# rlawhdrhs/Vision-Transformer-OpenCL

Hardware: AMD Instinct MI355X
Metric: images/sec ViT-B/16 224² fp32 @batch256; % MFMA roofline; top-1 match (higher is better)
Workload: dtype f32; 1 GPU; ViT-B/16 224x224 fp32 forward, batch 256 per GPU, synthetic weights and images (BASELINE.json configs[1]); batch_per_gpu=256, global_batch=256, parallelism=dp1, lanes_per_gpu=1, prune_last_layer=False, ln_fold=True, device=AMD Radeon Graphics, arch=gfx950:sramecc+:xnack-, compute_units=256, clock_mhz=2400

## Files before the change

### vision-transformer-opencl_amd/csrc/vit_gemm_common.hpp

```cpp
#pragma once
#include <hip/hip_runtime.h>

#include <type_traits>

#include "vit_hip_kernels.h"
#include "vit_split3.hpp"

namespace vitgemm {


typedef float f32x16 __attribute__((ext_vector_type(16)));
typedef float f32x4 __attribute__((ext_vector_type(4)));
typedef float f32x2 __attribute__((ext_vector_type(2)));
typedef unsigned u32x4 __attribute__((ext_vector_type(4)));

constexpr int KALIGN = 32;

enum { A_DENSE = 0, A_PATCHES = 1 };
enum { EPI_BIAS_LN = 3, EPI_BIAS_GELU_LN = 4, EPI_RESIDUAL_STATS = 5, EPI_BIAS_QGELU_LN = 7  };
constexpr bool epi_is_fold(int epi) { return epi == EPI_BIAS_LN || epi == EPI_BIAS_GELU_LN || epi == EPI_BIAS_QGELU_LN; }
constexpr bool epi_is_gelu(int epi) { return epi == VITHIP_EPI_BIAS_GELU || epi == EPI_BIAS_GELU_LN; }
constexpr bool epi_is_qgelu(int epi) { return epi == VITHIP_EPI_BIAS_QGELU || epi == EPI_BIAS_QGELU_LN; }

template <int... EPIS, typename F>
// ... 159 lines not shown
#pragma unroll
    for (int v = 0; v < NP; ++v) t[v] = f32x2{__builtin_amdgcn_rcpf(t[v].x), __builtin_amdgcn_rcpf(t[v].y)};
    __builtin_amdgcn_sched_barrier(0);
#pragma unroll
    for (int v = 0; v < NP; ++v) y[v] = y[v] * t[v];
}
__device__ __forceinline__ void quick_gelu_x8(float (&y)[8]) {
    f32x2 yy[4];
#pragma unroll
    for (int v = 0; v < 4; ++v) yy[v] = f32x2{y[2 * v], y[2 * v + 1]};
    quick_gelu_lockstep<4>(yy);
#pragma unroll
    for (int v = 0; v < 4; ++v) y[2 * v] = yy[v].x, y[2 * v + 1] = yy[v].y;
}

__device__ __forceinline__ int xcd_remap(int bid, int nwg) {
    const int q = nwg >> 3, rem = nwg & 7;
    const int xcd = bid & 7, idx = bid >> 3;
    const int base = xcd < rem ? xcd * (q + 1) : rem * (q + 1) + (xcd - rem) * q;
    return base + idx;
}

__device__ __forceinline__ void tile_coords(int tile, int tiles_m, int tiles_n, int group_m, int &tm, int &tn) {
    const int per_group = group_m * tiles_n;
    const int g = tile / per_group, in_g = tile - g * per_group;
    const int first = g * group_m;
    const int rows = tiles_m - first < group_m ? tiles_m - first : group_m;
    tn = in_g / rows;
    tm = first + (in_g - tn * rows);
}


enum { ARITH_F32 = 0, ARITH_SPLIT3 = 1 };
typedef __bf16 bf16x8 __attribute__((ext_vector_type(8)));
typedef __bf16 bf16x4 __attribute__((ext_vector_type(4)));
typedef unsigned u32x2 __attribute__((ext_vector_type(2)));
constexpr int SPLIT_BK = 16;
constexpr int SPLIT_LD = 28;
using vitsplit::SPLIT_TERM_A;
using vitsplit::SPLIT_TERM_W;
using vitsplit::bf16_to_f32;
using vitsplit::split3_piece;
using vitsplit::split3_piece2;
using vitsplit::split3_piece8;
__device__ __forceinline__ void split3_store(float *row, int kc, f32x4 x) {
#pragma unroll
    for (int piece = 0; piece < 3; ++piece) *reinterpret_cast<u32x2 *>(row + piece * 8 + kc / 2) = split3_piece(x, piece);
}

constexpr int WIMG_ROWS = 128;
constexpr int WIMG_BLOCK_BYTES = 3 * WIMG_ROWS * SPLIT_BK * 2;
constexpr int SPLIT_LD_SW = 32;
__device__ __forceinline__ int split_swizzle(int row) { return 2 * ((row & 3) ^ ((row >> 2) & 3)) + ((row >> 3) & 1); }
__device__ __forceinline__ int split_sw_offset(int row, int s) { return row * SPLIT_LD_SW + 4 * (s ^ split_swizzle(row)); }
template <int TM, int TN, int NS, typename Restage>
__device__ __forceinline__ void split3_step(f32x16 (&acc)[TM][TN], const float *As, const float *Bs, Restage &&restage) {
    bf16x8 a[TM][3], b[TN][3];
#pragma unroll
    for (int o = 0; o < 3; ++o) {
        const int pa = SPLIT_TERM_A[o], pb = SPLIT_TERM_W[o];
#pragma unroll
        for (int i = 0; i < TM; ++i) a[i][pa] = *reinterpret_cast<const bf16x8 *>(As + i * 32 * SPLIT_LD + pa * 8);
#pragma unroll
        for (int j = 0; j < TN; ++j) b[j][pb] = *reinterpret_cast<const bf16x8 *>(Bs + j * 32 * SPLIT_LD + pb * 8);
    }
    __builtin_amdgcn_sched_barrier(0);
    constexpr int NM = 6 * TM * TN, NR = NM / 2 > 0 ? NM / 2 : 1;
#pragma unroll
    for (int idx = 0; idx < NM; ++idx) {
        const int t = idx / (TM * TN), i = (idx / TN) % TM, j = idx % TN;
        acc[i][j] = __builtin_amdgcn_mfma_f32_32x32x16_bf16(a[i][SPLIT_TERM_A[t]], b[j][SPLIT_TERM_W[t]], acc[i][j], 0, 0, 0);
        if (idx < NR) {
            const int slot_before = (idx * NS) / NR, slot_after = ((idx + 1) * NS) / NR;
            if (slot_after > slot_before) {
                __builtin_amdgcn_sched_barrier(0);
#pragma unroll
                for (int q = slot_before; q < slot_after; ++q) restage(q);
                __builtin_amdgcn_sched_barrier(0);
            }
        }
    }
}

struct Split3PfRead { int w, piece, behind; };
constexpr int SPLIT_PF_BARRIER = 15;
constexpr Split3PfRead SPLIT_PF_READS[6] = {{0, 0, 15}, {1, 0, 16}, {1, 2, 17}, {0, 2, 18}, {0, 1, 19}, {1, 1, 20}};
struct Split3SlotsFine {
    static constexpr int N = 21;
    static constexpr int at(int q) {
        constexpr int gap[N] = {0, 1, 2, 3, 4, 4, 5, 6, 7, 8, 8, 9, 10, 12, 13, 1, 5, 9, 2, 6, 11};
        return gap[q];
    }
};
constexpr int split3_last_use(int w, int piece, int per_term) {
    int last = -1;
    for (int t = 0; t < 6; ++t)
        if ((w ? SPLIT_TERM_W[t] : SPLIT_TERM_A[t]) == piece) last = (t + 1) * per_term - 1;
    return last;
}
constexpr bool split3_pf_schedule_ok(int per_term) {
    for (int q = 0; q < Split3SlotsFine::N; ++q)
        if (Split3SlotsFine::at(q) < 0 || Split3SlotsFine::at(q) > SPLIT_PF_BARRIER) return false;
    bool seen[2][3] = {};
    for (int e = 0; e < 6; ++e) {
        const Split3PfRead rd = SPLIT_PF_READS[e];
        if (rd.behind < SPLIT_PF_BARRIER || rd.behind >= 6 * per_term) return false;
        if (rd.piece != 0 && rd.behind < split3_last_use(rd.w, rd.piece, per_term)) return false;
        if (e > 0 && rd.behind < SPLIT_PF_READS[e - 1].behind) return false;
        seen[rd.w][rd.piece] = true;
    }
    for (int w = 0; w < 2; ++w)
        for (int pc = 0; pc < 3; ++pc)
            if (!seen[w][pc]) return false;
    return true;
}
template <int TM, int TN>
struct Split3Frags {
    bf16x8 a[TM][3], b[TN][3];
    bf16x8 a_hn[TM], b_hn[TN];
};
template <int TM, int TN, bool NEXT>
__device__ __forceinline__ void split3_read_piece(Split3Frags<TM, TN> &f, const float *As, const float *Bs, const int (&poff)[3], int e) {
    const Split3PfRead rd = SPLIT_PF_READS[e];
    if (rd.w == 0) {
#pragma unroll
        for (int i = 0; i < TM; ++i) {
            const bf16x8 v = *reinterpret_cast<const bf16x8 *>(As + i * 32 * SPLIT_LD_SW + poff[rd.piece]);
            if (NEXT && rd.piece == 0) f.a_hn[i] = v;
            else f.a[i][rd.piece] = v;
        }
    } else {
#pragma unroll
        for (int j = 0; j < TN; ++j) {
            const bf16x8 v = *reinterpret_cast<const bf16x8 *>(Bs + j * 32 * SPLIT_LD_SW + poff[rd.piece]);
            if (NEXT && rd.piece == 0) f.b_hn[j] = v;
            else f.b[j][rd.piece] = v;
        }
    }
}
template <int TM, int TN>
__device__ __forceinline__ void split3_read_cold(Split3Frags<TM, TN> &f, const float *As, const float *Bs, const int (&poff)[3]) {
#pragma unroll
    for (int e = 0; e < 6; ++e) split3_read_piece<TM, TN, false>(f, As, Bs, poff, e);
}
struct Split3NoHook {
    __device__ __forceinline__ void operator()() const {}
};
template <int TM, int TN, bool PF, typename Restage, typename Sync, typename Landed = Split3NoHook>
__device__ __forceinline__ void split3_step_pf(f32x16 (&acc)[TM][TN], Split3Frags<TM, TN> &f, const float *An, const float *Bn,
                                               const int (&poff)[3], Restage &&restage, Sync &&sync, Landed &&landed = Landed{}) {
    constexpr int NM = 6 * TM * TN;
    static_assert(NM == 24, "the schedule table is laid out for 2 x 2 accumulators");
    static_assert(split3_pf_schedule_ok(TM * TN),
                  "restage writes in front of the barrier, reads of the other buffer behind it and behind the last use of what they overwrite");
    landed();
    __builtin_amdgcn_sched_barrier(0);
#pragma unroll
    for (int idx = 0; idx < NM; ++idx) {
        const int t = idx / (TM * TN), i = (idx / TN) % TM, j = idx % TN;
        acc[i][j] = __builtin_amdgcn_mfma_f32_32x32x16_bf16(f.a[i][SPLIT_TERM_A[t]], f.b[j][SPLIT_TERM_W[t]], acc[i][j], 0, 0, 0);
        __builtin_amdgcn_sched_barrier(0);
#pragma unroll
        for (int q = 0; q < Split3SlotsFine::N; ++q)
            if (Split3SlotsFine::at(q) == idx) restage(q);
        if (idx == SPLIT_PF_BARRIER) sync();
        if constexpr (PF) {
#pragma unroll
            for (int e = 0; e < 6; ++e)
                if (SPLIT_PF_READS[e].behind == idx) split3_read_piece<TM, TN, true>(f, An, Bn, poff, e);
        }
        __builtin_amdgcn_sched_barrier(0);
    }
    if constexpr (PF) {
#pragma unroll
        for (int i = 0; i < TM; ++i) f.a[i][0] = f.a_hn[i];
#pragma unroll
        for (int j = 0; j < TN; ++j) f.b[j][0] = f.b_hn[j];
    }
}

template <int TN, int TM = 1>
struct FoldOperands {
    float colsum[TN];
    const f32x2 *rows;
    float rstd[TM][16], mean[TM];
    bool preloaded;
};
template <int TN, int TM>
__device__ __forceinline__ void fold_preload(FoldOperands<TN, TM> &fold, const float *ln_rows, int M, int m_tile, int r, int h) {
#pragma unroll
    for (int i = 0; i < TM; ++i) {
        const int mr = m_tile + i * 32 + r;
        fold.mean[i] = ln_rows[2 * (size_t)(mr < M ? mr : M - 1) + 1];
#pragma unroll
        for (int v = 0; v < 16; ++v) {
            const int m = m_tile + i * 32 + 4 * h + (v & 3) + 8 * (v >> 2);
            fold.rstd[i][v] = ln_rows[2 * (size_t)(m < M ? m : M - 1)];
        }
    }
    fold.preloaded = true;
}
__device__ __forceinline__ float fold_center(float acc, float mean, float colsum) { return __builtin_fmaf(-mean, colsum, acc); }
__device__ __forceinline__ float fold_scale(float centered, float rstd, float bias) { return __builtin_fmaf(rstd, centered, bias); }

template <int BM, int BN, int WM, int WN, int EPI, int AMODE>
__device__ __forceinline__ void epilogue_store(const GemmParams &p, const f32x16 (&acc)[WM / 32][WN / 32],
                                               const float (&bias_r)[WN / 32], int m0, int n0, int wm, int wn,
                                               int r, int h, const FoldOperands<WN / 32, WM / 32> &fold = FoldOperands<WN / 32, WM / 32>{}) {
    constexpr int TM = WM / 32, TN = WN / 32;
    constexpr bool FOLD = epi_is_fold(EPI);
    constexpr bool GELU = epi_is_gelu(EPI), QGELU = epi_is_qgelu(EPI);
    constexpr int ST_NT = 2;
    const bool interior = (m0 + BM <= p.M) && (n0 + BN <= p.N);
    if (interior) {
        if constexpr (FOLD) {
            const __amdgpu_buffer_rsrc_t c_rsrc = __builtin_amdgcn_make_buffer_rsrc(p.C, 0, 0x7fffffff, 0x00020000);
            const bool center = p.ln_colsum != nullptr;
            auto rstd_of_block = [&](int i, float (&dst)[16]) __attribute__((always_inline)) {
#pragma unroll
                for (int g = 0; g < 4; ++g) {
                    const int lr = wm * WM + i * 32 + 4 * h + 8 * g;
#pragma unroll
                    for (int e = 0; e < 4; ++e) dst[4 * g + e] = fold.preloaded ? fold.rstd[i][4 * g + e] : fold.rows[lr + e].x;
                }
            };
            auto scale_and_store = [&](int i, const f32x16 (&src)[TN], const float (&row_rstd)[16]) __attribute__((always_inline)) {
                const int mb = m0 + wm * WM + i * 32 + 4 * h;
#pragma unroll
                for (int j = 0; j < TN; ++j) {
                    const int n = n0 + wn * WN + j * 32 + r;
                    const int c_off = (mb * p.ldc + n) * 4, c_row = p.ldc * 4;
#pragma unroll
                    for (int half = 0; half < 2; ++half) {
                        float y[8];
#pragma unroll
                        for (int q = 0; q < 8; ++q) y[q] = fold_scale(src[j][half * 8 + q], row_rstd[half * 8 + q], bias_r[j]);
                        if constexpr (GELU) gelu_erf_x8(y);
                        if constexpr (QGELU) quick_gelu_x8(y);
#pragma unroll
                        for (int q = 0; q < 8; ++q) {
                            const int v = half * 8 + q;
                            __builtin_amdgcn_raw_buffer_store_b32(__builtin_bit_cast(unsigned, y[q]), c_rsrc, c_off, ((v & 3) + 8 * (v >> 2)) * c_row, ST_NT);
                        }
                    }
                }
            };
            if (center) {
                float b_op[TN];
#pragma unroll
                for (int j = 0; j < TN; ++j) b_op[j] = h == 0 ? fold.colsum[j] : 0.0f;
#pragma unroll
                for (int i = 0; i < TM; ++i) {
                    const float mean = fold.preloaded ? fold.mean[i] : fold.rows[wm * WM + i * 32 + r].y;
                    const float a_op = h == 0 ? -mean : 0.0f;
                    f32x16 centered[TN];
#pragma unroll
                    for (int j = 0; j < TN; ++j) centered[j] = __builtin_amdgcn_mfma_f32_32x32x2f32(a_op, b_op[j], acc[i][j], 0, 0, 0);
                    float row_rstd[16];
                    rstd_of_block(i, row_rstd);
                    scale_and_store(i, centered, row_rstd);
// ... 215 lines not shown
```

### vision-transformer-opencl_amd/csrc/vit_gemm_persistent.hip

```cpp
#include "vit_device.hpp"
#include "vit_gemm_common.hpp"

namespace vitgemm {

constexpr int PBK = 32;
constexpr int PLD = PBK + 4;
constexpr int SK_HEADER_BYTES = 4096, SK_MAX_OWNERS = 1000, SK_STAT_TAKEN = 1016, SK_STAT_RECOMPUTED = 1017;

template <int BM, int BN, int WM, int WN, int EPI, bool STAMP = false, bool SK = false, int DBG = 0, int ARITH = ARITH_F32,
          bool WIMG = false>
__global__ __launch_bounds__(256, 2) void gemm_f32_nt_persistent_kernel(const GemmParams p) {
    constexpr bool SPLIT = ARITH == ARITH_SPLIT3;
    static_assert(!SPLIT || DBG == 0, "switch-off builds are fp32 only");
    static_assert(!WIMG || (SPLIT && BM == WIMG_ROWS && BN == WIMG_ROWS), "the weight image feeds the 128x128 split walk");
    constexpr bool PIPE = WIMG && EPI != VITHIP_EPI_BIAS_RESIDUAL && EPI != EPI_RESIDUAL_STATS;
    constexpr int PBK = SPLIT ? SPLIT_BK : vitgemm::PBK;
    constexpr int PLD = WIMG ? SPLIT_LD_SW : SPLIT ? SPLIT_LD : vitgemm::PLD;
    constexpr int ROWS_PER_PASS = 256 / (PBK / 4);
    constexpr int WGN = BN / WN;
    constexpr int TM = WM / 32, TN = WN / 32;
    constexpr int A_CHUNKS = BM * (PBK / 4) / 256;
    constexpr int B_CHUNKS = BN * (PBK / 4) / 256;
    constexpr int NC = PBK / 8;
    constexpr int NS = A_CHUNKS + B_CHUNKS;
    constexpr int W_CHUNKS = 3;
    constexpr int NL = WIMG ? A_CHUNKS + W_CHUNKS : NS;
    static_assert(!WIMG || (A_CHUNKS == 2 && BM * 2 == 256 && BN * 2 == 256), "WIMG: one 8-deep half row of A and of W per thread");
    constexpr int NM = 4 * TM * TN;
    static_assert((BM / WM) * WGN == 4, "4 waves per workgroup");

    __shared__ __attribute__((aligned(16))) float lds[2 * (BM + BN) * PLD];
    __shared__ int sk_decision;
    constexpr bool FOLD = epi_is_fold(EPI);
    __shared__ __attribute__((aligned(16))) f32x2 fold_rows_lds[FOLD ? 2 * BM : 2];
    static_assert(!FOLD || BM == 128, "one 16-byte lane copy of 64 lanes = 128 rows");
    float *const As0 = lds;
    float *const Bs0 = lds + 2 * BM * PLD;

    const int tid = threadIdx.x;
    const int lane = tid & 63, wave = tid >> 6;
    const int r = lane & 31, h = lane >> 5;
    const int wm = wave / WGN, wn = wave % WGN;

    unsigned long long st0 = 0, st_rt0 = 0, st_loop0 = 0, st_epi = 0;
    [[maybe_unused]] unsigned long long st_frag = 0, st_top = 0, st_landed = 0;
    auto stamp_top = [&]() __attribute__((always_inline)) {
        if constexpr (STAMP && WIMG) st_top = __builtin_amdgcn_s_memtime();
    };
    auto stamp_landed = [&]() __attribute__((always_inline)) {
        if constexpr (STAMP && WIMG) {
            __builtin_amdgcn_s_waitcnt(0xC07F);
            st_landed = __builtin_amdgcn_s_memtime();
        }
    };
    auto stamp_step = [&]() __attribute__((always_inline)) {
        if constexpr (STAMP && WIMG) st_frag += st_landed - st_top;
    };
    if constexpr (STAMP) {
        st0 = __builtin_amdgcn_s_memtime();
        st_rt0 = __builtin_amdgcn_s_memrealtime();
    }

    const int total = p.tiles_m * p.tiles_n;
    const int nwg = gridDim.x;
    const int first = xcd_remap(blockIdx.x, nwg);
    if (first >= total) return;
    const int nk = p.K / PBK;

    const int full = total / nwg, R = total - full * nwg;
    const int x = SK ? p.sk_x : 0;
    const int H = nwg - R;
    const bool owner = first < R;
    const int npre = (x > 0 && !owner && R > 0) ? (R - (first - R) + H - 1) / H : 0;
    const int pstart = (SK && p.sk_late) ? full : 0, fstart = (SK && p.sk_late) ? 0 : npre;
    const int nseg = npre + full + (owner ? 1 : 0);
    bool took = false;
    struct Seg { int tile, k0, k1, in, out; };
    auto get_seg = [&](int i) -> Seg {
        Seg g;
        if (i >= pstart && i < pstart + npre) {
            const int o = (first - R) + (i - pstart) * H;
            g.tile = full * nwg + o; g.k0 = 0; g.k1 = x; g.in = -1; g.out = o;
        } else if (i < npre + full) {
            g.tile = first + (i - fstart) * nwg; g.k0 = 0; g.k1 = nk; g.in = -1; g.out = -1;
        } else {
            g.tile = first + full * nwg; g.k0 = took ? x : 0; g.k1 = nk; g.in = took ? first : -1; g.out = -1;
        }
        return g;
    };

    const int ld_row = tid / (PBK / 4);
    const int ld_kc = (tid % (PBK / 4)) * 4;
    const int sw_row = tid >> 1, sw_half = tid & 1;
    int wr_off[3];
#pragma unroll
    for (int pl = 0; pl < 3; ++pl) wr_off[pl] = WIMG ? split_sw_offset(sw_row, 2 * pl + sw_half) : 0;
    const __amdgpu_buffer_rsrc_t a_rsrc = __builtin_amdgcn_make_buffer_rsrc(const_cast<float *>(p.A), 0, 0x7fffffff, 0x00020000);
    const __amdgpu_buffer_rsrc_t w_rsrc =
        __builtin_amdgcn_make_buffer_rsrc(const_cast<void *>(WIMG ? p.w_split : static_cast<const void *>(p.W)), 0, 0x7fffffff, 0x00020000);
    int a_src[A_CHUNKS];
    int b_src[WIMG ? W_CHUNKS : B_CHUNKS];
    f32x4 a_stage[A_CHUNKS], b_stage[B_CHUNKS];
    u32x4 w_stage[WIMG ? W_CHUNKS : 1];

    auto set_sources = [&](int tile) {
        int tm, tn;
        tile_coords(tile, p.tiles_m, p.tiles_n, p.group_m, tm, tn);
        if constexpr (WIMG) {
            int m = tm * BM + sw_row;
            m = m < p.M ? m : p.M - 1;
#pragma unroll
            for (int i = 0; i < A_CHUNKS; ++i) a_src[i] = (m * p.lda + 8 * sw_half + 4 * i) * 4;
#pragma unroll
            for (int q = 0; q < W_CHUNKS; ++q) b_src[q] = tn * nk * WIMG_BLOCK_BYTES + (q * 256 + tid) * 16;
            return;
        }
#pragma unroll
        for (int i = 0; i < A_CHUNKS; ++i) {
            int m = tm * BM + ld_row + i * ROWS_PER_PASS;
            m = m < p.M ? m : p.M - 1;
            a_src[i] = (m * p.lda + ld_kc) * 4;
        }
#pragma unroll
        for (int i = 0; i < B_CHUNKS; ++i) {
            int n = tn * BN + ld_row + i * ROWS_PER_PASS;
            n = n < p.N ? n : p.N - 1;
            b_src[i] = (n * p.ldw + ld_kc) * 4;
        }
    };
    auto load_bias = [&](int n0, float (&dst)[TN]) {
#pragma unroll
        for (int j = 0; j < TN; ++j) {
            const int n = n0 + wn * WN + j * 32 + r;
            dst[j] = n < p.N ? p.bias[n] : 0.0f;
        }
    };

    int *const sk_flags = reinterpret_cast<int *>(p.sk_ws);
    const int SK_PARKED = (p.sk_gen << 2) | 1, SK_WITHDRAWN = (p.sk_gen << 2) | 2;
    int steps = 0;
    auto decide = [&]() {
        if (tid == 0) {
            int *const f = sk_flags + first;
            int v = __hip_atomic_load(f, __ATOMIC_RELAXED, __HIP_MEMORY_SCOPE_AGENT);
            while (v != SK_PARKED) {
                int expected = v;
                if (__hip_atomic_compare_exchange_strong(f, &expected, SK_WITHDRAWN, __ATOMIC_RELAXED, __ATOMIC_RELAXED, __HIP_MEMORY_SCOPE_AGENT)) {
                    v = SK_WITHDRAWN;
                    break;
                }
                v = expected;
            }
            if (v == SK_PARKED) __hip_atomic_store(f, 0, __ATOMIC_RELAXED, __HIP_MEMORY_SCOPE_AGENT);
            __hip_atomic_fetch_add(sk_flags + (v == SK_PARKED ? SK_STAT_TAKEN : SK_STAT_RECOMPUTED), 1, __ATOMIC_RELAXED, __HIP_MEMORY_SCOPE_AGENT);
            sk_decision = v == SK_PARKED;
        }
        __syncthreads();
        took = __builtin_amdgcn_readfirstlane(sk_decision) != 0;
        if (took) steps -= x;
    };

    int seg_l = 0, k_l, kend_l;
    {
        const Seg g = get_seg(0);
        set_sources(g.tile);
        k_l = g.k0;
        kend_l = g.k1;
    }
    auto advance_load_cursor = [&]() {
        if (++k_l == kend_l) {
            if (++seg_l < nseg) {
                if (SK && owner && x > 0 && seg_l == nseg - 1) decide();
                const Seg g = get_seg(seg_l);
                set_sources(g.tile);
                k_l = g.k0;
                kend_l = g.k1;
            } else {
                k_l = kend_l - 1;
            }
        }
    };
    auto load_step = [&]() {
        const int k0 = k_l * PBK;
#pragma unroll
        for (int i = 0; i < A_CHUNKS; ++i) a_stage[i] = __builtin_bit_cast(f32x4, __builtin_amdgcn_raw_buffer_load_b128(a_rsrc, a_src[i], k0 * 4, 0));
        if constexpr (WIMG) {
#pragma unroll
            for (int q = 0; q < W_CHUNKS; ++q) w_stage[q] = __builtin_amdgcn_raw_buffer_load_b128(w_rsrc, b_src[q], k_l * WIMG_BLOCK_BYTES, 0);
            return;
        }
#pragma unroll
        for (int i = 0; i < B_CHUNKS; ++i) b_stage[i] = __builtin_bit_cast(f32x4, __builtin_amdgcn_raw_buffer_load_b128(w_rsrc, b_src[i], k0 * 4, 0));
    };
    auto stage_write = [&](float *row, f32x4 v) __attribute__((always_inline)) {
        if constexpr (SPLIT) split3_store(row, ld_kc, v);
        else *reinterpret_cast<f32x4 *>(row + ld_kc) = v;
    };
    auto write_a_plane = [&](float *As, int pl) __attribute__((always_inline)) {
        *reinterpret_cast<u32x4 *>(As + wr_off[pl]) = split3_piece8(a_stage[0], a_stage[1], pl);
    };
    auto write_w_plane = [&](float *Bs, int pl) __attribute__((always_inline)) { *reinterpret_cast<u32x4 *>(Bs + wr_off[pl]) = w_stage[pl]; };
    auto store_step = [&](int buf) {
        float *As = As0 + buf * BM * PLD, *Bs = Bs0 + buf * BN * PLD;
        if constexpr (WIMG) {
#pragma unroll
            for (int pl = 0; pl < 3; ++pl) {
                write_a_plane(As, pl);
                write_w_plane(Bs, pl);
            }
            return;
        }
#pragma unroll
        for (int i = 0; i < A_CHUNKS; ++i) stage_write(As + (ld_row + i * ROWS_PER_PASS) * PLD, a_stage[i]);
#pragma unroll
        for (int i = 0; i < B_CHUNKS; ++i) stage_write(Bs + (ld_row + i * ROWS_PER_PASS) * PLD, b_stage[i]);
    };
    auto restage_slot = [&](int q, int buf, int k0) {
        if (q < A_CHUNKS) {
            float *As = As0 + buf * BM * PLD;
            if (DBG != 5 && DBG != 6) stage_write(As + (ld_row + q * ROWS_PER_PASS) * PLD, a_stage[q]);
            if (DBG != 2 && DBG != 6) a_stage[q] = __builtin_bit_cast(f32x4, __builtin_amdgcn_raw_buffer_load_b128(a_rsrc, a_src[q], k0 * 4, 0));
        } else {
            const int qb = q - A_CHUNKS;
            float *Bs = Bs0 + buf * BN * PLD;
            if (DBG != 5 && DBG != 6) stage_write(Bs + (ld_row + qb * ROWS_PER_PASS) * PLD, b_stage[qb]);
            if (DBG != 2 && DBG != 6) b_stage[qb] = __builtin_bit_cast(f32x4, __builtin_amdgcn_raw_buffer_load_b128(w_rsrc, b_src[qb], k0 * 4, 0));
        }
    };

    u32x4 a_plane;
    auto restage_fine = [&](int q, int buf, int k0) {
        if (q <= 12) {
            const int pl = q / 5, sub = q % 5;
            auto quarter = [&](int s4) __attribute__((always_inline)) {
                f32x4 &x = a_stage[s4 >> 1];
                const int o = 2 * (s4 & 1);
                f32x2 xx = {x[o], x[o + 1]};
                unsigned pc = split3_piece2(xx, pl);
                asm volatile("" : "+v"(pc), "+v"(xx));
                x[o] = xx[0];
                x[o + 1] = xx[1];
                a_plane[s4] = pc;
            };
            if (pl < 2 && sub < 4) quarter(sub);
            else if (pl == 2 && sub < 2) {
                quarter(2 * sub);
                quarter(2 * sub + 1);
            } else *reinterpret_cast<u32x4 *>(As0 + buf * BM * PLD + wr_off[pl]) = a_plane;
        } else if (q <= 14) {
            a_stage[q - 13] = __builtin_bit_cast(f32x4, __builtin_amdgcn_raw_buffer_load_b128(a_rsrc, a_src[q - 13], k0 * 4, 0));
        } else if (q <= 17) {
            write_w_plane(Bs0 + buf * BN * PLD, q - 15);
        } else {
            w_stage[q - 18] = __builtin_amdgcn_raw_buffer_load_b128(w_rsrc, b_src[q - 18], (k0 / PBK) * WIMG_BLOCK_BYTES, 0);
        }
    };
    auto restage_any = [&](int q, int buf, int k0) __attribute__((always_inline)) {
        restage_fine(q, buf, k0);
    };

    const int a_frag_off = WIMG ? (wm * WM + r) * PLD : (wm * WM + r) * PLD + h * 4;
    const int b_frag_off = WIMG ? (wn * WN + r) * PLD : (wn * WN + r) * PLD + h * 4;
    int frag_poff[3];
#pragma unroll
    for (int pc = 0; pc < 3; ++pc) frag_poff[pc] = WIMG ? split_sw_offset(r, 2 * pc + h) - r * PLD : 0;
    f32x4 af[2][TM], bf[2][TN];
    auto read_frags = [&](int buf, int c, int set) {
        if constexpr (SPLIT) return;
        const float *As = As0 + buf * BM * PLD + a_frag_off + c * 8;
        const float *Bs = Bs0 + buf * BN * PLD + b_frag_off + c * 8;
#pragma unroll
        for (int i = 0; i < TM; ++i) af[set][i] = *reinterpret_cast<const f32x4 *>(As + i * 32 * PLD);
#pragma unroll
        for (int j = 0; j < TN; ++j) bf[set][j] = *reinterpret_cast<const f32x4 *>(Bs + j * 32 * PLD);
    };

    f32x16 acc[TM][TN];
    constexpr int SC_SYS = 0x11;
    auto slot_rsrc = [&](int o) {
        return __builtin_amdgcn_make_buffer_rsrc(reinterpret_cast<char *>(p.sk_ws) + SK_HEADER_BYTES + (size_t)o * (BM * BN * 4), 0, BM * BN * 4, 0x00020000);
    };
    auto park = [&](int o) {
        const __amdgpu_buffer_rsrc_t rs = slot_rsrc(o);
#pragma unroll
        for (int i = 0; i < TM; ++i)
#pragma unroll
            for (int j = 0; j < TN; ++j)
#pragma unroll
                for (int q4 = 0; q4 < 4; ++q4) {
                    f32x4 v;
#pragma unroll
                    for (int e = 0; e < 4; ++e) v[e] = acc[i][j][4 * q4 + e];
                    __builtin_amdgcn_raw_buffer_store_b128(__builtin_bit_cast(u32x4, v), rs, tid * 16,
                                                           ((i * TN + j) * 4 + q4) * 4096, SC_SYS);
                }
        asm volatile("s_waitcnt vmcnt(0)" ::: "memory");
        __syncthreads();
        if (tid == 0) {
            int cur = __hip_atomic_load(sk_flags + o, __ATOMIC_RELAXED, __HIP_MEMORY_SCOPE_AGENT);
            for (;;) {
                if (cur == SK_WITHDRAWN) {
                    __hip_atomic_store(sk_flags + o, 0, __ATOMIC_RELAXED, __HIP_MEMORY_SCOPE_AGENT);
                    break;
                }
                int expected = cur;
                if (__hip_atomic_compare_exchange_strong(sk_flags + o, &expected, SK_PARKED, __ATOMIC_RELAXED, __ATOMIC_RELAXED, __HIP_MEMORY_SCOPE_AGENT)) break;
                cur = expected;
            }
        }
    };
    auto unpark = [&](int o) {
        const __amdgpu_buffer_rsrc_t rs = slot_rsrc(o);
#pragma unroll
        for (int i = 0; i < TM; ++i)
#pragma unroll
            for (int j = 0; j < TN; ++j)
#pragma unroll
                for (int q4 = 0; q4 < 4; ++q4) {
                    const f32x4 v = __builtin_bit_cast(f32x4, __builtin_amdgcn_raw_buffer_load_b128(rs, tid * 16, ((i * TN + j) * 4 + q4) * 4096, SC_SYS));
#pragma unroll
                    for (int e = 0; e < 4; ++e) acc[i][j][4 * q4 + e] = v[e];
                }
        __builtin_amdgcn_s_waitcnt(0x0F70);
    };

    int seg_c = 0, k_c, kend_c, m0, n0, out_c;
    [[maybe_unused]] int seg_k0 = 0;
    float bias_r[TN];
    FoldOperands<TN, TM> fold{};
    [[maybe_unused]] int fold_buf = 0;
    auto begin_segment = [&](int i) {
        const Seg g = get_seg(i);
        int tm, tn;
        tile_coords(g.tile, p.tiles_m, p.tiles_n, p.group_m, tm, tn);
        m0 = tm * BM;
        n0 = tn * BN;
        k_c = g.k0;
        seg_k0 = g.k0;
        kend_c = g.k1;
        out_c = g.out;
        if (g.out < 0) load_bias(n0, bias_r);
        if constexpr (FOLD) {
            if (g.out < 0) {
#pragma unroll
                for (int j = 0; j < TN; ++j) {
                    const int n = n0 + wn * WN + j * 32 + r;
                    fold.colsum[j] = (p.ln_colsum && n < p.N) ? p.ln_colsum[n] : 0.0f;
                }
                if (wave == 0) {
                    const int left = p.M - m0 < BM ? p.M - m0 : BM;
                    const __amdgpu_buffer_rsrc_t rr = __builtin_amdgcn_make_buffer_rsrc(const_cast<float *>(p.ln_rows) + (size_t)m0 * 2, 0, left * 8, 0x00020000);
                    const unsigned dst = (unsigned)(size_t)(fold_rows_lds + fold_buf * BM);
                    asm volatile("s_mov_b32 m0, %0\n\ts_nop 0\n\tbuffer_load_dwordx4 %1, %2, 0 offen lds" ::"s"(dst), "v"(lane * 16), "s"(rr) : "memory", "m0");
                }
                fold.rows = fold_rows_lds + fold_buf * BM;
                fold_buf ^= 1;
            }
        }
        if (SK && g.in >= 0) {
            unpark(g.in);
        } else {
#pragma unroll
            for (int ii = 0; ii < TM; ++ii)
#pragma unroll
                for (int jj = 0; jj < TN; ++jj)
#pragma unroll
                    for (int v = 0; v < 16; ++v) acc[ii][jj][v] = 0.0f;
        }
    };
    begin_segment(0);

    for (int i = 0; i < nseg; ++i) {
        const Seg g = get_seg(i);
        steps += g.k1 - g.k0;
    }
    load_step();
    advance_load_cursor();
    store_step(0);
    load_step();
    advance_load_cursor();
    __syncthreads();
    read_frags(0, 0, 0);
    if (DBG == 4) read_frags(0, 1, 1);
    (void)af; (void)bf;

    auto end_segment = [&]() {
        unsigned long long e0 = 0;
        if constexpr (STAMP) e0 = __builtin_amdgcn_s_memtime();
        if (SK && out_c >= 0) park(out_c);
        else if (DBG != 1 || p.M < 0) {
            if constexpr (EPI == EPI_RESIDUAL_STATS) epilogue_store_residual_stats<BM, BN, WM, WN>(p, acc, bias_r, m0, n0, wm, wn, r, h);
            else epilogue_store<BM, BN, WM, WN, EPI, A_DENSE>(p, acc, bias_r, m0, n0, wm, wn, r, h, fold);
        }
        if constexpr (STAMP) st_epi += __builtin_amdgcn_s_memtime() - e0;
        if (++seg_c < nseg) begin_segment(seg_c);
    };
    auto fold_rows_landed = [&]() {
        if constexpr (FOLD) {
            if (out_c < 0) {
                constexpr int FOLD_WAIT = 2 * NL, FOLD_MIN_STEPS = 4;
                static_assert(FOLD_WAIT <= 63, "vmcnt is a 6-bit count on gfx950");
                static_assert((FOLD_MIN_STEPS - 1) * NL >= FOLD_WAIT + NL, "the copy must be older than the loads the wait leaves in flight");
                if (kend_c - seg_k0 >= FOLD_MIN_STEPS) asm volatile("s_waitcnt vmcnt(%0)" ::"n"(FOLD_WAIT) : "memory");
                else asm volatile("s_waitcnt vmcnt(0)" ::: "memory");
            }
        }
    };

    if constexpr (STAMP) st_loop0 = __builtin_amdgcn_s_memtime();
    int cur = 0;
    if constexpr (PIPE) {
        Split3Frags<TM, TN> frags;
        auto tile_a = [&](int buf) { return As0 + buf * BM * PLD + a_frag_off; };
        auto tile_b = [&](int buf) { return Bs0 + buf * BN * PLD + b_frag_off; };
        auto step = [&](auto prefetch) __attribute__((always_inline)) {
            constexpr bool PF = decltype(prefetch)::value;
            const int k_ahead = k_l * PBK;
            split3_step_pf<TM, TN, PF>(acc, frags, tile_a(cur ^ 1), tile_b(cur ^ 1), frag_poff,
                [&](int q) __attribute__((always_inline)) { restage_any(q, cur ^ 1, k_ahead); }, [] { __syncthreads(); }, stamp_landed);
            stamp_step();
            stamp_top();
            advance_load_cursor();
            cur ^= 1;
            ++k_c;
        };
        for (;;) {
            stamp_top();
            split3_read_cold<TM, TN>(frags, tile_a(cur), tile_b(cur), frag_poff);
            while (k_c + 1 < kend_c) step(std::true_type{});
            fold_rows_landed();
            step(std::false_type{});
            end_segment();
            if (seg_c >= nseg) break;
        }
    } else
    for (int g = 0; g < steps; ++g) {
        const int k_ahead = k_l * PBK;
        if (k_c + 1 == kend_c) fold_rows_landed();
        if constexpr (WIMG) {
            Split3Frags<TM, TN> frags;
            stamp_top();
            split3_read_cold<TM, TN>(frags, As0 + cur * BM * PLD + a_frag_off, Bs0 + cur * BN * PLD + b_frag_off, frag_poff);
            split3_step_pf<TM, TN, false>(acc, frags, nullptr, nullptr, frag_poff,
                [&](int q) __attribute__((always_inline)) { restage_fine(q, cur ^ 1, k_ahead); }, [] {}, stamp_landed);
            stamp_step();
            advance_load_cursor();
            __syncthreads();
        } else if constexpr (SPLIT) {
            split3_step<TM, TN, NS>(acc, As0 + cur * BM * PLD + a_frag_off, Bs0 + cur * BN * PLD + b_frag_off,
                                    [&](int q) __attribute__((always_inline)) { restage_slot(q, cur ^ 1, k_ahead); });
            advance_load_cursor();
            __syncthreads();
        } else
#pragma unroll
        for (int c = 0; c < NC; ++c) {
            if (c + 1 < NC && DBG != 4) read_frags(cur, c + 1, (c + 1) & 1);
            if (c == NC - 1) {
                if (DBG != 3) __syncthreads();
                if (DBG != 4) read_frags(cur ^ 1, 0, NC & 1);
            }
            __builtin_amdgcn_sched_barrier(0);
#pragma unroll
            for (int idx = 0; idx < NM; ++idx) {
                const int s2 = idx / (TM * TN), i = (idx / TN) % TM, j = idx % TN;
                acc[i][j] = __builtin_amdgcn_mfma_f32_32x32x2f32(af[c & 1][i][s2], bf[c & 1][j][s2], acc[i][j], 0, 0, 0);
                if (c == 0) {
                    const int slot_before = (idx * NS) / NM, slot_after = ((idx + 1) * NS) / NM;
                    if (slot_after > slot_before) {
                        __builtin_amdgcn_sched_barrier(0);
#pragma unroll
                        for (int q = slot_before; q < slot_after; ++q) restage_slot(q, cur ^ 1, k_ahead);
                        __builtin_amdgcn_sched_barrier(0);
                    }
                }
            }
            if (c == 0) advance_load_cursor();
        }
        cur ^= 1;

        if (++k_c == kend_c) end_segment();
    }
    if constexpr (STAMP) {
        const unsigned long long c3 = __builtin_amdgcn_s_memtime(), r3 = __builtin_amdgcn_s_memrealtime();
        if (tid == 0) {
            unsigned long long *d = p.dbg + (size_t)blockIdx.x * 8;
            d[0] = st0; d[1] = st_loop0; d[2] = st_epi; d[3] = c3; d[4] = WIMG ? st_frag : st_rt0; d[5] = r3;
            d[6] = (unsigned long long)nseg; d[7] = (unsigned long long)steps;
        }
    }
}

static int persistent_wgs() { return 2 * vitdev::current_cus(); }

int persistent_piece_steps(int M, int N, int K, int slots, int wgs, int kstep) {
    if (wgs <= 0) wgs = persistent_wgs();
    if (wgs <= 0) return 0;
    const int total = ((M + 127) / 128) * ((N + 127) / 128);
    const int nwg = total < wgs ? total : wgs;
    const int full = total / nwg, R = total - full * nwg, nk = K / PBK;
    if (full < 1 || R <= 0 || R >= nwg || R > slots || R > SK_MAX_OWNERS) return 0;
    const int c = (R + (nwg - R) - 1) / (nwg - R);
    const int x = nk / (c + 1);
    return (x >= 4 && nk - c * x >= 8) ? x * (PBK / kstep) : 0;
}

template <int BM, int BN, int WM, int WN, int ARITH = ARITH_F32, bool WIMG = false>
int launch_persistent_tile(hipStream_t stream, GemmParams &p, int epilogue, int group_m) {
    const int wgs = persistent_wgs();
    if (wgs <= 0) return static_cast<int>(hipErrorInvalidDevice);
    const dim3 grid(set_tile_grid(p, BM, BN, wgs)), block(256);
    p.group_m = group_m;
    p.sk_x = (p.sk_ws && BM == 128 && BN == 128) ? persistent_piece_steps(p.M, p.N, p.K, p.sk_slots, wgs, ARITH == ARITH_SPLIT3 ? SPLIT_BK : PBK) : 0;
    return with_epilogue(WalkEpilogues{}, epilogue, [&](auto epi) {
        auto launch = [&](auto sk) {
            hipLaunchKernelGGL((gemm_f32_nt_persistent_kernel<BM, BN, WM, WN, decltype(epi)::value, false, decltype(sk)::value, 0, ARITH, WIMG>), grid, block, 0, stream, p);
            return static_cast<int>(hipGetLastError());
        };
        return p.sk_x > 0 ? launch(std::true_type{}) : launch(std::false_type{});
    });
}

#ifdef VIT_PROBES
template <int EPI, bool STAMP, int DBG = 0, int ARITH = ARITH_F32, bool WIMG = false>
static int launch_walk_probe(hipStream_t stream, GemmParams &p, int group_m) {
    const int wgs = persistent_wgs();
    if (wgs <= 0) return static_cast<int>(hipErrorInvalidDevice);
    const dim3 grid(set_tile_grid(p, 128, 128, wgs));
    p.group_m = group_m;
    p.sk_x = 0;
    hipLaunchKernelGGL((gemm_f32_nt_persistent_kernel<128, 128, 64, 64, EPI, STAMP, false, DBG, ARITH, WIMG>), grid, dim3(256), 0, stream, p);
    return static_cast<int>(hipGetLastError());
// ... 38 lines not shown
```

Before: 5507 images/sec.

## Load pre-split weight fragments straight from global memory into registers, bypassing LDS

In the WIMG split3 GEMM path, the pre-split bf16 weight fragments are now read by each lane directly from global memory into MFMA operand registers. They are no longer staged through LDS and read back. This drops the W half of the LDS buffers, the W LDS writes and reads, and their restage slots, and schedules the six per-step W loads between MFMAs one k-step ahead. The trade is more in-flight global loads per lane and exposure to memory latency without LDS sharing across waves, in exchange for less LDS traffic and footprint.

```diff
diff --git a/vision-transformer-opencl_amd/csrc/vit_gemm_common.hpp b/vision-transformer-opencl_amd/csrc/vit_gemm_common.hpp
--- a/vision-transformer-opencl_amd/csrc/vit_gemm_common.hpp
+++ b/vision-transformer-opencl_amd/csrc/vit_gemm_common.hpp
@@ -265,13 +265,15 @@
     }
 }
 
-struct Split3PfRead { int w, piece, behind; };
+struct Split3PfRead { int piece, behind; };
 constexpr int SPLIT_PF_BARRIER = 15;
-constexpr Split3PfRead SPLIT_PF_READS[6] = {{0, 0, 15}, {1, 0, 16}, {1, 2, 17}, {0, 2, 18}, {0, 1, 19}, {1, 1, 20}};
+constexpr Split3PfRead SPLIT_PF_READS[3] = {{0, 15}, {2, 17}, {1, 19}};
+struct Split3WLoad { int piece, j, behind; };
+constexpr Split3WLoad SPLIT_W_LOADS[6] = {{0, 0, 1}, {0, 1, 2}, {2, 0, 5}, {2, 1, 6}, {1, 0, 16}, {1, 1, 18}};
 struct Split3SlotsFine {
-    static constexpr int N = 21;
+    static constexpr int N = 15;
     static constexpr int at(int q) {
-        constexpr int gap[N] = {0, 1, 2, 3, 4, 4, 5, 6, 7, 8, 8, 9, 10, 12, 13, 1, 5, 9, 2, 6, 11};
+        constexpr int gap[N] = {0, 1, 2, 3, 4, 4, 5, 6, 7, 8, 8, 9, 10, 12, 13};
         return gap[q];
     }
 };
@@ -281,61 +283,67 @@
         if ((w ? SPLIT_TERM_W[t] : SPLIT_TERM_A[t]) == piece) last = (t + 1) * per_term - 1;
     return last;
 }
-constexpr bool split3_pf_schedule_ok(int per_term) {
+constexpr bool split3_pf_schedule_ok(int per_term, int blocks_w) {
     for (int q = 0; q < Split3SlotsFine::N; ++q)
         if (Split3SlotsFine::at(q) < 0 || Split3SlotsFine::at(q) > SPLIT_PF_BARRIER) return false;
-    bool seen[2][3] = {};
-    for (int e = 0; e < 6; ++e) {
+    bool seen[3] = {};
+    for (int e = 0; e < 3; ++e) {
         const Split3PfRead rd = SPLIT_PF_READS[e];
         if (rd.behind < SPLIT_PF_BARRIER || rd.behind >= 6 * per_term) return false;
-        if (rd.piece != 0 && rd.behind < split3_last_use(rd.w, rd.piece, per_term)) return false;
+        if (rd.piece != 0 && rd.behind < split3_last_use(0, rd.piece, per_term)) return false;
         if (e > 0 && rd.behind < SPLIT_PF_READS[e - 1].behind) return false;
-        seen[rd.w][rd.piece] = true;
-    }
-    for (int w = 0; w < 2; ++w)
-        for (int pc = 0; pc < 3; ++pc)
-            if (!seen[w][pc]) return false;
-    return true;
+        seen[rd.piece] = true;
+    }
+    for (int pc = 0; pc < 3; ++pc)
+        if (!seen[pc]) return false;
+    int asked = 0;
+    for (int e = 0; e < 6; ++e) {
+        const Split3WLoad ld = SPLIT_W_LOADS[e];
+        if (ld.piece < 0 || ld.piece > 2 || ld.j < 0 || ld.j >= blocks_w) return false;
+        if (ld.behind < 0 || ld.behind >= 6 * per_term) return false;
+        if (ld.piece != 0 && ld.behind < split3_last_use(1, ld.piece, per_term)) return false;
+        if (e > 0 && ld.behind < SPLIT_W_LOADS[e - 1].behind) return false;
+        asked |= 1 << (ld.piece * blocks_w + ld.j);
+    }
+    return asked == (1 << (3 * blocks_w)) - 1;
 }
 template <int TM, int TN>
 struct Split3Frags {
     bf16x8 a[TM][3], b[TN][3];
     bf16x8 a_hn[TM], b_hn[TN];
 };
+template <int TM, int TN>
+__device__ __forceinline__ bf16x8 &split3_w_dst(Split3Frags<TM, TN> &f, int piece, int j) {
+    return piece != 0 ? f.b[j][piece] : f.b_hn[j];
+}
 template <int TM, int TN, bool NEXT>
-__device__ __forceinline__ void split3_read_piece(Split3Frags<TM, TN> &f, const float *As, const float *Bs, const int (&poff)[3], int e) {
+__device__ __forceinline__ void split3_read_piece(Split3Frags<TM, TN> &f, const float *As, const int (&poff)[3], int e) {
     const Split3PfRead rd = SPLIT_PF_READS[e];
-    if (rd.w == 0) {
-#pragma unroll
-        for (int i = 0; i < TM; ++i) {
-            const bf16x8 v = *reinterpret_cast<const bf16x8 *>(As + i * 32 * SPLIT_LD_SW + poff[rd.piece]);
-            if (NEXT && rd.piece == 0) f.a_hn[i] = v;
-            else f.a[i][rd.piece] = v;
-        }
-    } else {
-#pragma unroll
-        for (int j = 0; j < TN; ++j) {
-            const bf16x8 v = *reinterpret_cast<const bf16x8 *>(Bs + j * 32 * SPLIT_LD_SW + poff[rd.piece]);
-            if (NEXT && rd.piece == 0) f.b_hn[j] = v;
-            else f.b[j][rd.piece] = v;
-        }
+#pragma unroll
+    for (int i = 0; i < TM; ++i) {
+        const bf16x8 v = *reinterpret_cast<const bf16x8 *>(As + i * 32 * SPLIT_LD_SW + poff[rd.piece]);
+        if (NEXT && rd.piece == 0) f.a_hn[i] = v;
+        else f.a[i][rd.piece] = v;
     }
 }
 template <int TM, int TN>
-__device__ __forceinline__ void split3_read_cold(Split3Frags<TM, TN> &f, const float *As, const float *Bs, const int (&poff)[3]) {
-#pragma unroll
-    for (int e = 0; e < 6; ++e) split3_read_piece<TM, TN, false>(f, As, Bs, poff, e);
+__device__ __forceinline__ void split3_read_cold(Split3Frags<TM, TN> &f, const float *As, const int (&poff)[3]) {
+#pragma unroll
+    for (int e = 0; e < 3; ++e) split3_read_piece<TM, TN, false>(f, As, poff, e);
 }
 struct Split3NoHook {
     __device__ __forceinline__ void operator()() const {}
 };
-template <int TM, int TN, bool PF, typename Restage, typename Sync, typename Landed = Split3NoHook>
-__device__ __forceinline__ void split3_step_pf(f32x16 (&acc)[TM][TN], Split3Frags<TM, TN> &f, const float *An, const float *Bn,
-                                               const int (&poff)[3], Restage &&restage, Sync &&sync, Landed &&landed = Landed{}) {
+template <int TM, int TN, bool PFA, bool PFW, typename Restage, typename LoadW, typename Sync, typename Landed = Split3NoHook>
+__device__ __forceinline__ void split3_step_pf(f32x16 (&acc)[TM][TN], Split3Frags<TM, TN> &f, const float *An, const int (&poff)[3],
+                                               Restage &&restage, LoadW &&load_w, Sync &&sync, Landed &&landed = Landed{}) {
     constexpr int NM = 6 * TM * TN;
     static_assert(NM == 24, "the schedule table is laid out for 2 x 2 accumulators");
-    static_assert(split3_pf_schedule_ok(TM * TN),
-                  "restage writes in front of the barrier, reads of the other buffer behind it and behind the last use of what they overwrite");
+    static_assert(split3_pf_schedule_ok(TM * TN, TN),
+                  "A: restage writes in front of the barrier, reads of the other buffer behind it and behind the last use of what they "
+                  "overwrite; W: every fragment requested once, mid and lo behind their last use");
+#pragma unroll
+    for (int j = 0; j < TN; ++j) f.b[j][0] = f.b_hn[j];
     landed();
     __builtin_amdgcn_sched_barrier(0);
 #pragma unroll
@@ -343,22 +351,25 @@
         const int t = idx / (TM * TN), i = (idx / TN) % TM, j = idx % TN;
         acc[i][j] = __builtin_amdgcn_mfma_f32_32x32x16_bf16(f.a[i][SPLIT_TERM_A[t]], f.b[j][SPLIT_TERM_W[t]], acc[i][j], 0, 0, 0);
         __builtin_amdgcn_sched_barrier(0);
+        if constexpr (PFW) {
+#pragma unroll
+            for (int e = 0; e < 6; ++e)
+                if (SPLIT_W_LOADS[e].behind == idx) split3_w_dst(f, SPLIT_W_LOADS[e].piece, SPLIT_W_LOADS[e].j) = load_w(SPLIT_W_LOADS[e].piece, SPLIT_W_LOADS[e].j);
+        }
 #pragma unroll
         for (int q = 0; q < Split3SlotsFine::N; ++q)
             if (Split3SlotsFine::at(q) == idx) restage(q);
         if (idx == SPLIT_PF_BARRIER) sync();
-        if constexpr (PF) {
-#pragma unroll
-            for (int e = 0; e < 6; ++e)
-                if (SPLIT_PF_READS[e].behind == idx) split3_read_piece<TM, TN, true>(f, An, Bn, poff, e);
+        if constexpr (PFA) {
+#pragma unroll
+            for (int e = 0; e < 3; ++e)
+                if (SPLIT_PF_READS[e].behind == idx) split3_read_piece<TM, TN, true>(f, An, poff, e);
         }
         __builtin_amdgcn_sched_barrier(0);
     }
-    if constexpr (PF) {
+    if constexpr (PFA) {
 #pragma unroll
         for (int i = 0; i < TM; ++i) f.a[i][0] = f.a_hn[i];
-#pragma unroll
-        for (int j = 0; j < TN; ++j) f.b[j][0] = f.b_hn[j];
     }
 }
 
diff --git a/vision-transformer-opencl_amd/csrc/vit_gemm_persistent.hip b/vision-transformer-opencl_amd/csrc/vit_gemm_persistent.hip
--- a/vision-transformer-opencl_amd/csrc/vit_gemm_persistent.hip
+++ b/vision-transformer-opencl_amd/csrc/vit_gemm_persistent.hip
@@ -23,19 +23,19 @@
     constexpr int B_CHUNKS = BN * (PBK / 4) / 256;
     constexpr int NC = PBK / 8;
     constexpr int NS = A_CHUNKS + B_CHUNKS;
-    constexpr int W_CHUNKS = 3;
-    constexpr int NL = WIMG ? A_CHUNKS + W_CHUNKS : NS;
-    static_assert(!WIMG || (A_CHUNKS == 2 && BM * 2 == 256 && BN * 2 == 256), "WIMG: one 8-deep half row of A and of W per thread");
+    constexpr int W_FRAGS = 3 * TN;
+    constexpr int NL = WIMG ? A_CHUNKS + W_FRAGS : NS;
+    static_assert(!WIMG || (A_CHUNKS == 2 && BM * 2 == 256), "WIMG: one 8-deep half row of A per thread");
     constexpr int NM = 4 * TM * TN;
     static_assert((BM / WM) * WGN == 4, "4 waves per workgroup");
 
-    __shared__ __attribute__((aligned(16))) float lds[2 * (BM + BN) * PLD];
+    __shared__ __attribute__((aligned(16))) float lds[2 * (WIMG ? BM : BM + BN) * PLD];
     __shared__ int sk_decision;
     constexpr bool FOLD = epi_is_fold(EPI);
     __shared__ __attribute__((aligned(16))) f32x2 fold_rows_lds[FOLD ? 2 * BM : 2];
     static_assert(!FOLD || BM == 128, "one 16-byte lane copy of 64 lanes = 128 rows");
     float *const As0 = lds;
-    float *const Bs0 = lds + 2 * BM * PLD;
+    float *const Bs0 = WIMG ? lds : lds + 2 * BM * PLD;
 
     const int tid = threadIdx.x;
     const int lane = tid & 63, wave = tid >> 6;
@@ -49,7 +49,7 @@
     };
     auto stamp_landed = [&]() __attribute__((always_inline)) {
         if constexpr (STAMP && WIMG) {
-            __builtin_amdgcn_s_waitcnt(0xC07F);
+            __builtin_amdgcn_s_waitcnt(0x0074);
             st_landed = __builtin_amdgcn_s_memtime();
         }
     };
@@ -99,9 +99,10 @@
     const __amdgpu_buffer_rsrc_t w_rsrc =
         __builtin_amdgcn_make_buffer_rsrc(const_cast<void *>(WIMG ? p.w_split : static_cast<const void *>(p.W)), 0, 0x7fffffff, 0x00020000);
     int a_src[A_CHUNKS];
-    int b_src[WIMG ? W_CHUNKS : B_CHUNKS];
+    int b_src[B_CHUNKS];
     f32x4 a_stage[A_CHUNKS], b_stage[B_CHUNKS];
-    u32x4 w_stage[WIMG ? W_CHUNKS : 1];
+    const int w_lane = WIMG ? ((wn * WN + r) * 2 + h) * 16 : 0;
+    [[maybe_unused]] int w_panel = 0;
 
     auto set_sources = [&](int tile) {
         int tm, tn;
@@ -111,8 +112,6 @@
             m = m < p.M ? m : p.M - 1;
 #pragma unroll
             for (int i = 0; i < A_CHUNKS; ++i) a_src[i] = (m * p.lda + 8 * sw_half + 4 * i) * 4;
-#pragma unroll
-            for (int q = 0; q < W_CHUNKS; ++q) b_src[q] = tn * nk * WIMG_BLOCK_BYTES + (q * 256 + tid) * 16;
             return;
         }
 #pragma unroll
@@ -184,11 +183,7 @@
         const int k0 = k_l * PBK;
 #pragma unroll
         for (int i = 0; i < A_CHUNKS; ++i) a_stage[i] = __builtin_bit_cast(f32x4, __builtin_amdgcn_raw_buffer_load_b128(a_rsrc, a_src[i], k0 * 4, 0));
-        if constexpr (WIMG) {
-#pragma unroll
-            for (int q = 0; q < W_CHUNKS; ++q) w_stage[q] = __builtin_amdgcn_raw_buffer_load_b128(w_rsrc, b_src[q], k_l * WIMG_BLOCK_BYTES, 0);
-            return;
-        }
+        if constexpr (WIMG) return;
 #pragma unroll
         for (int i = 0; i < B_CHUNKS; ++i) b_stage[i] = __builtin_bit_cast(f32x4, __builtin_amdgcn_raw_buffer_load_b128(w_rsrc, b_src[i], k0 * 4, 0));
     };
@@ -199,15 +194,11 @@
     auto write_a_plane = [&](float *As, int pl) __attribute__((always_inline)) {
         *reinterpret_cast<u32x4 *>(As + wr_off[pl]) = split3_piece8(a_stage[0], a_stage[1], pl);
     };
-    auto write_w_plane = [&](float *Bs, int pl) __attribute__((always_inline)) { *reinterpret_cast<u32x4 *>(Bs + wr_off[pl]) = w_stage[pl]; };
     auto store_step = [&](int buf) {
         float *As = As0 + buf * BM * PLD, *Bs = Bs0 + buf * BN * PLD;
         if constexpr (WIMG) {
 #pragma unroll
-            for (int pl = 0; pl < 3; ++pl) {
-                write_a_plane(As, pl);
-                write_w_plane(Bs, pl);
-            }
+            for (int pl = 0; pl < 3; ++pl) write_a_plane(As, pl);
             return;
         }
 #pragma unroll
@@ -247,20 +238,20 @@
                 quarter(2 * sub);
                 quarter(2 * sub + 1);
             } else *reinterpret_cast<u32x4 *>(As0 + buf * BM * PLD + wr_off[pl]) = a_plane;
-        } else if (q <= 14) {
+        } else {
             a_stage[q - 13] = __builtin_bit_cast(f32x4, __builtin_amdgcn_raw_buffer_load_b128(a_rsrc, a_src[q - 13], k0 * 4, 0));
-        } else if (q <= 17) {
-            write_w_plane(Bs0 + buf * BN * PLD, q - 15);
-        } else {
-            w_stage[q - 18] = __builtin_amdgcn_raw_buffer_load_b128(w_rsrc, b_src[q - 18], (k0 / PBK) * WIMG_BLOCK_BYTES, 0);
-        }
+        }
+    };
+    auto load_w_frag = [&](int pl, int j, int k) __attribute__((always_inline)) {
+        return __builtin_bit_cast(bf16x8, __builtin_amdgcn_raw_buffer_load_b128(w_rsrc, w_lane + j * (32 * 2 * 16),
+                                                                                 w_panel + k * WIMG_BLOCK_BYTES + pl * (WIMG_ROWS * 2 * 16), 0));
     };
     auto restage_any = [&](int q, int buf, int k0) __attribute__((always_inline)) {
         restage_fine(q, buf, k0);
     };
 
     const int a_frag_off = WIMG ? (wm * WM + r) * PLD : (wm * WM + r) * PLD + h * 4;
-    const int b_frag_off = WIMG ? (wn * WN + r) * PLD : (wn * WN + r) * PLD + h * 4;
+    const int b_frag_off = (wn * WN + r) * PLD + h * 4;
     int frag_poff[3];
 #pragma unroll
     for (int pc = 0; pc < 3; ++pc) frag_poff[pc] = WIMG ? split_sw_offset(r, 2 * pc + h) - r * PLD : 0;
@@ -335,6 +326,7 @@
         tile_coords(g.tile, p.tiles_m, p.tiles_n, p.group_m, tm, tn);
         m0 = tm * BM;
         n0 = tn * BN;
+        if constexpr (WIMG) w_panel = tn * nk * WIMG_BLOCK_BYTES;
         k_c = g.k0;
         seg_k0 = g.k0;
         kend_c = g.k1;
@@ -409,24 +401,34 @@
 
     if constexpr (STAMP) st_loop0 = __builtin_amdgcn_s_memtime();
     int cur = 0;
-    if constexpr (PIPE) {
+    if constexpr (WIMG) {
         Split3Frags<TM, TN> frags;
         auto tile_a = [&](int buf) { return As0 + buf * BM * PLD + a_frag_off; };
-        auto tile_b = [&](int buf) { return Bs0 + buf * BN * PLD + b_frag_off; };
         auto step = [&](auto prefetch) __attribute__((always_inline)) {
             constexpr bool PF = decltype(prefetch)::value;
             const int k_ahead = k_l * PBK;
-            split3_step_pf<TM, TN, PF>(acc, frags, tile_a(cur ^ 1), tile_b(cur ^ 1), frag_poff,
-                [&](int q) __attribute__((always_inline)) { restage_any(q, cur ^ 1, k_ahead); }, [] { __syncthreads(); }, stamp_landed);
+            if constexpr (!PIPE) split3_read_cold<TM, TN>(frags, tile_a(cur), frag_poff);
+            split3_step_pf<TM, TN, PF && PIPE, PF>(acc, frags, tile_a(cur ^ 1), frag_poff,
+                [&](int q) __attribute__((always_inline)) { restage_any(q, cur ^ 1, k_ahead); },
+                [&](int pl, int j) __attribute__((always_inline)) { return load_w_frag(pl, j, k_c + 1); },
+                [] { if constexpr (PIPE) __syncthreads(); }, stamp_landed);
             stamp_step();
-            stamp_top();
+            if constexpr (PIPE) stamp_top();
             advance_load_cursor();
+            if constexpr (!PIPE) {
+                __syncthreads();
+                stamp_top();
+            }
             cur ^= 1;
             ++k_c;
         };
         for (;;) {
             stamp_top();
-            split3_read_cold<TM, TN>(frags, tile_a(cur), tile_b(cur), frag_poff);
+#pragma unroll
+            for (int e = 0; e < 6; ++e)
+                split3_w_dst(frags, SPLIT_W_LOADS[e].piece, SPLIT_W_LOADS[e].j) = load_w_frag(SPLIT_W_LOADS[e].piece, SPLIT_W_LOADS[e].j, k_c);
+            if constexpr (PIPE) split3_read_cold<TM, TN>(frags, tile_a(cur), frag_poff);
+            __builtin_amdgcn_s_waitcnt(0x0F70);
             while (k_c + 1 < kend_c) step(std::true_type{});
             fold_rows_landed();
             step(std::false_type{});
@@ -437,16 +439,7 @@
     for (int g = 0; g < steps; ++g) {
         const int k_ahead = k_l * PBK;
         if (k_c + 1 == kend_c) fold_rows_landed();
-        if constexpr (WIMG) {
-            Split3Frags<TM, TN> frags;
-            stamp_top();
-            split3_read_cold<TM, TN>(frags, As0 + cur * BM * PLD + a_frag_off, Bs0 + cur * BN * PLD + b_frag_off, frag_poff);
-            split3_step_pf<TM, TN, false>(acc, frags, nullptr, nullptr, frag_poff,
-                [&](int q) __attribute__((always_inline)) { restage_fine(q, cur ^ 1, k_ahead); }, [] {}, stamp_landed);
-            stamp_step();
-            advance_load_cursor();
-            __syncthreads();
-        } else if constexpr (SPLIT) {
+        if constexpr (SPLIT) {
             split3_step<TM, TN, NS>(acc, As0 + cur * BM * PLD + a_frag_off, Bs0 + cur * BN * PLD + b_frag_off,
                                     [&](int q) __attribute__((always_inline)) { restage_slot(q, cur ^ 1, k_ahead); });
             advance_load_cursor();
```

Measured after the change: 5653 images/sec, median of 6. +2.6%, better.
